# johannesulf/TabCorr

Hardware: AMD Instinct MI355X
Metric: predict_calls_per_sec (higher is better)
Workload: dtype f64; 1 GPU; BASELINE configs[1]: Zheng07 predict(), synthetic auto table 50 mass bins x {cen,sat} (G=100, P=5050), 19 rp bins, n_gauss_prim=10, batch of 10000 draws per GPU per step, draws and results resident in HBM; n_tables=1, gather=none, gather_payload=ngal + xi (160 B per draw), gather_every_steps=32, lanes=4, rccl_ranks=0

## Files before the change

tabcorr_amd/csrc/hostmath.cpp:

```cpp
#include "hostmath.h"
#include "fastmath.h"
#include "series.h"

#include <algorithm>
#include <atomic>
#include <cmath>
#include <cstring>
#include <map>
#include <numeric>
#include <tuple>
#include <thread>

namespace tc {

void gauss_legendre(int n, std::vector<double>& x, std::vector<double>& w) {
  x.assign(n, 0.0);
  w.assign(n, 0.0);
  const long double pi = 3.141592653589793238462643383279502884L;
  for (int i = 0; i < (n + 1) / 2; ++i) {
    long double z = cosl(pi * (i + 0.75L) / (n + 0.5L));
    long double dp = 1.0L;
    for (int iter = 0; iter < 100; ++iter) {
      long double p0 = 1.0L, p1 = z;
      for (int k = 2; k <= n; ++k) {
// ... 704 lines not shown
}

void triangle_parts(int n_rb, int n_parts, int32_t* rb0, int32_t* cb0, int32_t* count) {
  const int64_t n_units = (int64_t)n_rb * (n_rb + 1) / 2;
  for (int part = 0; part < n_parts; ++part) {
    const int64_t begin = n_units * part / n_parts, end = n_units * (part + 1) / n_parts;
    int64_t rb = (int64_t)((std::sqrt(8.0 * (double)begin + 1.0) - 1.0) / 2.0);
    while ((rb + 1) * (rb + 2) / 2 <= begin) ++rb;
    while (rb * (rb + 1) / 2 > begin) --rb;
    rb0[part] = (int32_t)rb;
    cb0[part] = (int32_t)(begin - rb * (rb + 1) / 2);
    count[part] = (int32_t)(end - begin);
  }
}

QuadTiling quad_tiling(int n_r) {
  QuadTiling tiling;
  tiling.n_rtiles = (n_r + 19) / 20;
  tiling.r_per_tile = (n_r + tiling.n_rtiles - 1) / tiling.n_rtiles;
  tiling.n_u = (tiling.r_per_tile + 3) / 4;
  return tiling;
}

void fill_quad_table(const QuadLayout& layout, const std::vector<int32_t>& perm, int n_r,
                     int64_t n_pairs, const void* matrix, bool matrix_is_f32,
                     const QuadTiling& tiling, std::vector<double>& out) {
  const int up = (tiling.n_u + 1) / 2;
  const size_t per_unit = (size_t)up * 128;
  out.assign((size_t)tiling.n_rtiles * layout.n_units * per_unit, 0.0);
  auto source = [&](int r, int64_t column) {
// ... 478 lines not shown
```

tabcorr_amd/csrc/hostmath.h:

```cpp
#pragma once

#include <cstdint>
#include <string>
#include <vector>

namespace tc {

void gauss_legendre(int n, std::vector<double>& x, std::vector<double>& w);

inline int64_t packed_index(int64_t i, int64_t j) {
  return i >= j ? i * (i + 1) / 2 + j : j * (j + 1) / 2 + i;
}

bool spline_interpolation_matrix(int n, const double* xp, std::vector<double>& a);

struct Segment {
  int32_t component;
  int32_t rectangular;
  int32_t i_lo, i_hi;
  int32_t j_lo, j_hi;
  int64_t q_begin;
  int64_t n_real;
};

// ... 114 lines not shown
  int32_t pad;
};
struct QuadMergePlan {
  int waves_per_block = 0;
  int n_blocks = 0;
  int lds_slots = 0;
  std::vector<int32_t> block_begin;
  std::vector<QuadMerge> merges;
};
void merge_quad_schedule(const QuadLayout& layout, int n_rtiles, bool separate,
                         int waves_per_block, int max_slots, QuadSchedule& schedule,
                         QuadMergePlan& plan);

void triangle_parts(int n_rb, int n_parts, int32_t* rb0, int32_t* cb0, int32_t* count);

struct QuadTiling {
  int n_rtiles = 1;
  int r_per_tile = 0;
  int n_u = 0;
};
QuadTiling quad_tiling(int n_r);

void fill_quad_table(const QuadLayout& layout, const std::vector<int32_t>& perm, int n_r,
                     int64_t n_pairs, const void* matrix, bool matrix_is_f32,
                     const QuadTiling& tiling, std::vector<double>& out);

QuadTiling quad_tiling_f32(int n_r);
void fill_quad_table_f32(const QuadLayout& layout, const std::vector<int32_t>& perm, int n_r,
                         int64_t n_pairs, const void* matrix, bool matrix_is_f32,
                         const QuadTiling& tiling, std::vector<float>& out);
// ... 47 lines not shown
```

tabcorr_amd/csrc/inst_fused.hip:

```cpp
#include "inst_fused.h"

namespace tc {
namespace host {

int launch_fused_instance(const FusedInstance& in, int device, int n_u, dim3 grid, dim3 block,
                       int lds, hipStream_t stream, hipEvent_t k0, hipEvent_t k1,
                       const tc::FusedArgs& fa) {
  const bool assembias = in.assembias, modulate = in.modulate;
  if (in.draws == 40) return launch_fused_instance_40(in, TC_FUSED_ARGS);
  if (in.draws == 32) return launch_fused_instance_32(in, TC_FUSED_ARGS);
  if (in.waves == 16) return launch_fused_instance_16(in, TC_FUSED_ARGS);
#define TC_FUSED(NG, AB, MO, LE) launch_fused<NG, AB, MO, LE, 8>(TC_FUSED_ARGS)
#define TC_FUSED_GROUPED(AB, MO) launch_fused<10, AB, MO, false, 8, 64, true>(TC_FUSED_ARGS)
  if (in.grouped)
    return assembias ? (modulate ? TC_FUSED_GROUPED(true, true) : TC_FUSED_GROUPED(true, false))
                     : (modulate ? TC_FUSED_GROUPED(false, true) : TC_FUSED_GROUPED(false, false));
  if (in.leauthaud) return modulate ? TC_FUSED(0, false, true, true) : TC_FUSED(0, false, false, true);
  if (in.n_gauss != 10) return TC_FUSED(0, false, false, false);
  if (!assembias && !modulate && in.defer == 2)
    return launch_fused<10, false, false, false, 8, 64, false, 2>(TC_FUSED_ARGS);
  if (!assembias && !modulate && in.defer == 1)
    return launch_fused<10, false, false, false, 8, 64, false, 1>(TC_FUSED_ARGS);
  if (!assembias && !modulate) return TC_FUSED(10, false, false, false);
  if (!assembias) return TC_FUSED(10, false, true, false);
  if (!modulate) return TC_FUSED(10, true, false, false);
  return TC_FUSED(10, true, true, false);
#undef TC_FUSED
#undef TC_FUSED_GROUPED
}

}
}
```

tabcorr_amd/csrc/internal.h:

```cpp
#pragma once

#include <hip/hip_runtime.h>
#include <hip/hip_ext.h>

#include <algorithm>
#include <chrono>
#include <cmath>
#include <cstdarg>
#include <cstdio>
#include <cstdlib>
#include <cstring>
#include <map>
#include <memory>
#include <string>
#include <utility>
#include <vector>

#include "../../include/tabcorr_amd.h"
#include "../../include/tabcorr_amd_testing.h"
#include "fastmath.h"
#include "hostmath.h"
#include "kernel_args.h"

namespace tc {
// ... 217 lines not shown
  int occ_splits = 0;
  int occ_per_cu = 4;
  int n_groups = 0, n_waves = 0, lds_min = 0, min_chunk_entries = 32;
  int k_splits = 0;
  int trace = 0;
  int autotune_after = 0;
  int sync_chunks = 0;
  int sync_form = 32;
  int sync_stagger = 10;
  int sync_direct_out = 2;
  int async_direct_in = 1;
  int async_direct_out = 2;
  int series = -1;
  int cross_defer = 1;
  int fused_defer = 2;
  int fused_sat_cap = 6;
  int cross_wide_min_draws = 4096;
  int cross_target = 160;
  int resident_aperture = 1;
  int cross_min_draws = 192;
  int fused = 1;
  int fused_min_draws = 0;
  int fused_max_draws = 30720;
  int fused_waves = 0;
  int fused_draws = 0;
  int fused_spread = 1, fused_spread_min = 8192, fused_spread_rounds = 1;
  int prio_fused = 1, prio_fused_occ = 2, prio_fused_out = 3;
  int deterministic = 0;
  int skip_occ = 0, skip_finalize = 0;
  void load() {
// ... 65 lines not shown
  int compute_dtype = TC_DTYPE_F64;
  bool legacy = false;
  tc::Plan plan;
  int rt = 0;
  int n_rtiles = 0;
  hipStream_t stream = nullptr;
  hipEvent_t ev_begin = nullptr, ev_end = nullptr;

  std::vector<double> n_h, log_min, log_max, percentile, dist_index;

  void* d_table = nullptr;
  size_t table_bytes = 0;
  void* d_n_h = nullptr;
  void* d_percentile = nullptr;
  void* d_perm = nullptr;
  tc::NodeGroups node_groups;
  void* d_group_begin = nullptr;
  void* d_group_member = nullptr;
  void* d_group_n_h = nullptr;
  void* d_group_percentile = nullptr;
  bool grouped = false;
  void* d_math_table = nullptr;
  void* d_pos_ij = nullptr;
  void* d_pos_off = nullptr;
  std::vector<double> cross_host;
  tc::host::CrossFused cross_fused, cross_fused_wide;
  int sync_cross_target = 0;
  std::vector<hipEvent_t> chunk_events;
  bool sync_spread = false;
  bool quad = false;
// ... 5 lines not shown
  std::map<unsigned, AutoChoice> autotuned;
  std::map<unsigned, int> pipelined_calls;
  bool autotuning = false;
  std::map<int, tc::host::Quadrature> quadrature;
  std::map<std::pair<int, int>, std::unique_ptr<tc::host::DeviceChunking>> chunkings;
  std::map<int64_t, tc::host::DeviceChunking*> choices;

  struct Lane {
    hipStream_t stream = nullptr;
    hipEvent_t finished = nullptr;
    tc::host::DeviceBuffer nbuf, ngal2, partial;
    tc::host::DeviceBuffer nbuf32;
    tc::host::DeviceBuffer xi;
    tc::host::DeviceBuffer in_theta, out;
    tc::host::DeviceBuffer cross_counters;
    int ngal_parts = 1;
  };
  static constexpr int kMaxLanes = 8;
  Lane lanes[kMaxLanes];
  int n_lanes = 2;
  int prev = -1;
  int cur = 0;
  int force_lane = -1;
  int async_lane = -1;
  bool chain = false;
  struct Ticket {
    hipEvent_t done = nullptr;
    int64_t id = -1;
  };
  static constexpr int kMaxTickets = 64;
// ... 161 lines not shown
int launch_occupation(const tc::OccArgs& oa, unsigned flags, int n_gauss, bool grouped,
                      int64_t grid_blocks, hipStream_t stream);
int launch_occ_from_array_kernel(const double* occupation_device, int64_t n_draws, int64_t ldb,
                                 int n_bins, int n_central, const double* n_h,
                                 const int32_t* perm, double* nbuf, double* ngal2, float* nbuf32,
                                 hipStream_t stream);
struct FusedInstance {
  int n_gauss = 10;
  bool assembias = false, modulate = false, leauthaud = false, grouped = false;
  int waves = 8, draws = 64;
  int defer = 0;
};
int launch_fused_instance(const FusedInstance& instance, int device, int n_u, dim3 grid,
                          dim3 block, int lds, hipStream_t stream, hipEvent_t k0, hipEvent_t k1,
                          const tc::FusedArgs& fa);
int launch_cross_instance(bool assembias, bool modulate, bool defer, int device, int rows,
                          dim3 grid, dim3 block, int lds, hipStream_t stream, hipEvent_t k0,
                          hipEvent_t k1, const tc::CrossFusedArgs& ca);
int launch_single_kernel(int blocks, hipStream_t stream, const tc::SingleArgs& sa);
int launch_resident_kernel(int blocks, hipStream_t stream, const tc::SingleArgs& sa);
int launch_ensemble_kernel(int device, int grid, int lds_bytes, hipStream_t stream,
                           const tc::EnsembleArgs& ea);

int copy_in(PinnedBuffer* stage, void* device, const void* host, size_t bytes,
            hipStream_t stream);
int copy_out(PinnedBuffer* stage, double* ngal, size_t ngal_count, const void* d_ngal,
             double* xi, size_t xi_count, const void* d_xi, hipStream_t stream);

}
}
// ... 1 lines not shown
```

tabcorr_amd/csrc/kernel_args.h:

```cpp
#pragma once

#include <cstdint>

#include "hostmath.h"

namespace tc {

constexpr int kLanes = 64;
constexpr unsigned kFlagSeparate = 1u;
constexpr unsigned kFlagModulate = 2u;
constexpr unsigned kFlagAssembias = 4u;
constexpr int kOccWaves = 4;
constexpr int kF32Block = 8;
constexpr int kF64Block = 8;
constexpr int kF32Tile = 32;
constexpr int kFinalizeRows = 32;
constexpr int kMaxInterpDim = 8;
constexpr int kMaxInterpAxis = 32;

struct GroupArgs {
  const int32_t* begin;
  const int32_t* member;
  const double* log_m;
  const double* m;
// ... 245 lines not shown
  uint32_t table_bytes;
  double* ngal;
  double* xi;
  const double* chi2_data;
  double* chi2;
  int n_groups;
  int n_central_groups;
  GroupArgs group;
  const double* series;
  const int32_t* series_thr;
  const double* sat_series;
  const int32_t* sat_series_thr;
  int sat_cap;
  const double* sat_records;
  const double* cen_records;
};

constexpr int kCrossWaves = 8;
constexpr int kCrossChunkBins = 48;
constexpr int kCrossMaxRows = 128;
constexpr int kCrossTableDoubles = 2306;
constexpr int kCrossSmallRows = 16, kCrossSmallChunk = 8;
constexpr int kCrossMaxSplits = 8;
constexpr int cross_small_lds_doubles(int n_comp) {
  return kCrossTableDoubles + kCrossWaves * kCrossSmallChunk * kLanes +
         n_comp * kCrossSmallRows * kLanes;
}
constexpr int cross_buffer_doubles(int rows) {
  return 2 * kCrossChunkBins * kLanes > rows * kLanes ? 2 * kCrossChunkBins * kLanes
                                                      : rows * kLanes;
// ... 87 lines not shown
```

tabcorr_amd/csrc/kernels.hip.h:

```cpp
#pragma once

#include <hip/hip_runtime.h>

#include <cstdint>
#include <utility>

#include "fastmath.h"
#include "hostmath.h"
#include "kernel_args.h"
#include "series.h"

#ifdef TC_DEVELOPER_KNOBS
#define TC_TRACE(pointer) ((pointer) != nullptr)
#else
#define TC_TRACE(pointer) false
#endif

namespace tc {

static_assert(sizeof(QuadRun) == 32 && sizeof(QuadCompArgs) == 32, "read as 8 x int32");

typedef const __attribute__((address_space(4))) double* sc_f64;
typedef const __attribute__((address_space(4))) float* sc_f32;
typedef const __attribute__((address_space(4))) int32_t* sc_i32;
// ... 1807 lines not shown
    }
    for (int idx = threadIdx.x; idx < rows * kLanes; idx += blockDim.x) {
      const int d = idx / rows, rr = idx % rows;
      if (d < n_valid) a.xi[(col + d) * (int64_t)n_rows + row0 + rr] = tile[rr][d];
    }
    __syncthreads();
  }
}

constexpr int fused_slot_doubles(int waves, int draws = 64) {
  return waves * 4 * kQuadMaxU * (draws == 40 ? 40 : kQuadTile);
}
__device__ __forceinline__ constexpr int dens40(int row, int draw) {
  return row * 40 + (draw & 3) * 10 + (draw >> 2);
}
constexpr int fused_scratch_doubles(int waves) { return fm::kTableDoubles + 2 * waves * kLanes; }
static_assert(kFusedWaves == 8 && kFusedMaxParts == 8, "8 or 16 waves: 4 or 8 parts per tile");
static_assert(20 * (kLanes + 1) + 20 * 21 <= fm::kTableDoubles,
              "results tile + likelihood data in the place of the math table");

template <int UU, int DL>
__device__ __forceinline__ void fused_quad_pass(__amdgpu_buffer_rsrc_t rs_t, unsigned off_a,
                                                unsigned unit_bytes, const double* dens_b,
                                                const double* dens_e, int rb, int cb, int left,
                                                bool triangular, int n_cb, unsigned unit_base,
                                                double (&F)[2][2]) {
  unsigned ua = (unit_base + (unsigned)(triangular ? rb * (rb + 1) / 2 + cb : rb * n_cb + cb)) *
                unit_bytes;
  f64x2 t0, t1, b0, b1;
  f64x4 D[UU][2];
  auto fetch = [&](f64x2& t, f64x2& b, int column) {
// ... 66 lines not shown
__device__ __forceinline__ int wave_prefix_sum(int value) {
  auto shifted = [](int x, auto control, auto rows) {
    return __builtin_amdgcn_update_dpp(0, x, decltype(control)::value, decltype(rows)::value, 0xf,
                                       false);
  };
  typedef std::integral_constant<int, 0xf> all_rows;
  value += shifted(value, std::integral_constant<int, 0x111>(), all_rows());
  value += shifted(value, std::integral_constant<int, 0x112>(), all_rows());
  value += shifted(value, std::integral_constant<int, 0x114>(), all_rows());
  value += shifted(value, std::integral_constant<int, 0x118>(), all_rows());
  value += shifted(value, std::integral_constant<int, 0x142>(), std::integral_constant<int, 0xa>());
  value += shifted(value, std::integral_constant<int, 0x143>(), std::integral_constant<int, 0xc>());
  return value;
}

__device__ __forceinline__ double fused_quad_rows40(double select, double value, double sums) {
  return __builtin_amdgcn_mfma_f64_4x4x4f64(select, value, sums, 0, 0, 0);
}

template <int S0, int NS>
__device__ __forceinline__ void fused_quad_pass40(__amdgpu_buffer_rsrc_t rs_t, unsigned off_a,
                                                  unsigned unit_bytes, const double* dens_b,
                                                  const double* dens_e, int rb, int cb, int left,
                                                  bool triangular, int n_cb, unsigned unit_base,
                                                  double (&F)[NS][10]) {
  unsigned ua = (unit_base + (unsigned)(triangular ? rb * (rb + 1) / 2 + cb : rb * n_cb + cb)) *
                unit_bytes;
  double ta[2][NS];
  f64x2 tb[2][5];
  double D[NS][10];
// ... 86 lines not shown

template <int NGAUSS, int U, bool ASSEMBIAS, bool MODULATE, bool LEAUTHAUD = false,
          int W = kFusedWaves, int DL = 64, bool GROUPED = false, int SATDEFER = 0>
__global__ __launch_bounds__(64 * W, DL == 40 ? 2 : W == 8 ? (SATDEFER == 2 ? 4 : 2) : 1) void predict_fused_kernel(
    FusedArgs a) {
  static_assert(!SATDEFER || (NGAUSS == 10 && !ASSEMBIAS && !MODULATE && !LEAUTHAUD && DL != 32 &&
                              !GROUPED), "deferred pairs");
  static_assert(!GROUPED || (NGAUSS == 10 && !LEAUTHAUD), "groups of bins: Zheng07, ten nodes");
  static_assert((DL == 64 && (W == 8 || W == 16)) || ((DL == 32 || DL == 40) && W == 8),
                "workgroup shape");
  static_assert(DL == 64 || NGAUSS == 10 || LEAUTHAUD, "32 / 40 draws: ten nodes per bin");
  static_assert(DL != 40 || (!ASSEMBIAS && !MODULATE && !LEAUTHAUD && !GROUPED), "latency form");
  constexpr int PARTS = DL == 40 ? W : W * 32 / DL;
  static_assert(!LEAUTHAUD || (NGAUSS == 0 && !ASSEMBIAS), "Leauthaud11: any n_gauss, undecorated");
  constexpr int UP = (U + 1) / 2;
  extern __shared__ __attribute__((aligned(16))) double fused_lds[];
  constexpr int kSlotDoubles = fused_slot_doubles(W, DL);
  const int region_b = a.dens_rows * DL > kSlotDoubles ? a.dens_rows * DL : kSlotDoubles;
  double* dens = fused_lds;
  double* table = fused_lds + region_b;
  double(*red)[W][kLanes] = (double(*)[W][kLanes])(table + fm::kTableDoubles);
  const fm::Consts kc = fm::make_consts();
#ifdef TC_DEVELOPER_KNOBS
  const int skip = (a.priority >> 8) & 3;
  const int n_bins_occ = (skip & 1) ? 0 : a.n_bins;
  unsigned long long* const stamps =
      ((a.priority >> 10) & 1) && a.chi2 == nullptr ? (unsigned long long*)a.chi2_data : nullptr;
  auto wave_stamp = [&](int which) {
    if (stamps != nullptr && (threadIdx.x & 63) == 0 && W == 8 && ((threadIdx.x >> 6) & 3) == 0)
      stamps[blockIdx.x * 32 + 16 + 8 * (threadIdx.x >> 8) + which] =
          __builtin_amdgcn_s_memrealtime();
  };
  auto stamp = [&](int which) {
    if (stamps != nullptr && threadIdx.x == 0)
      stamps[blockIdx.x * 32 + which] = __builtin_amdgcn_s_memrealtime();
  };
// ... 7 lines not shown
#endif
  stamp(0);
  set_priority((a.priority >> 2) & 3);
  const int lane = threadIdx.x & 63;
  const int wave = __builtin_amdgcn_readfirstlane(threadIdx.x >> 6);
  const int n_gauss = NGAUSS > 0 ? NGAUSS : a.n_gauss;
  {
    typedef double __attribute__((ext_vector_type(2))) double2v;
    const int hi = fm::kTableDoubles / 2;
    const double2v* src = (const double2v*)a.math_table;
    double2v* dst = (double2v*)table;
    for (int i = threadIdx.x; i < hi; i += blockDim.x) dst[i] = src[i];
  }
  for (int idx = a.n_bins * DL + threadIdx.x; idx < a.dens_rows * DL; idx += blockDim.x)
    dens[idx] = 0.0;
  __syncthreads();
  stamp(1);

  const int draw = DL != 32 ? lane : (lane & 31);
  const int half = DL != 32 ? 0 : (lane >> 5);
  const bool live = DL != 40 || lane < 40;
  auto dens_at = [&](int row, int d) -> double& {
    return dens[DL == 40 ? dens40(row, d) : row * DL + d];
  };
  const int64_t col = (int64_t)blockIdx.x * DL;
  const int64_t b0 = col + draw;
  const int64_t b = b0 < a.n_draws ? b0 : a.n_draws - 1;
  double norm;
  {
    const double* th = a.theta + b * a.n_theta;
    LeauthaudDraw ld;
    if (LEAUTHAUD) ld = prepare_leauthaud(table, kc, th);
    const DrawSetup d =
        LEAUTHAUD ? prepare_draw(table, kc, 12.0, 1.0, 12.0, 13.0, 1.0, 0.0, 0.0)
                  : prepare_draw(table, kc, th[0], th[1], th[2], th[3], th[4],
                                 ASSEMBIAS ? th[5] : 0.0, ASSEMBIAS ? th[6] : 0.0);
    DrawParams dp;
    dp.log_m_min = d.log_m_min;
    dp.inv_sigma = d.inv_sigma;
    dp.m0 = d.m0;
    dp.log2_m1 = d.log2_m1;
    dp.sat_scale = d.sat_scale;
// ... 27 lines not shown
          const double value = acc * n_h_m[mi];
          if (half == 0) dens[g * DL + draw] = value;
          if (central) sum_cen += value; else sum_sat += value;
        };
        if (DL == 32)
          occ_group_zheng07_halves<ASSEMBIAS, MODULATE>(
              table, kc, gr, group_begin[gr], group_begin[gr + 1], central, half, a.group.log_m,
              a.group.m, a.group.weight, gq, a.split, dp, emit);
        else
          occ_group_zheng07<ASSEMBIAS, MODULATE>(table, kc, gr, group_begin[gr],
                                                 group_begin[gr + 1], central, gq, a.split, dp,
                                                 emit);
      }
    }
    unsigned mine = 0;
    for (int g = wave; g < (GROUPED ? 0 : n_bins_occ); g += W) {
      const bool central = g < a.n_central;
      const bool above = ASSEMBIAS ? percentile[g] > a.split : false;
      bool deferred = false;
      const double acc =
          SATDEFER == 2 && central
              ? occ_cen_record(table, kc,
                               (sc_f64)a.cen_records + g * series::cen_record::kStride, dp,
                               &deferred) :
          SATDEFER && !central && (SATDEFER == 2 || a.sat_cap == series::sat::kShortest)
              ? occ_sat_record(table, kc,
                               (sc_f64)a.sat_records + g * series::sat_record::kStride, dp,
                               &deferred) :
          DL == 32 && LEAUTHAUD
              ? occ_bin_leauthaud11_halves<MODULATE>(table, kc, g, central, half, a.log_m, a.m,
// ... 2 lines not shown
                                                                    half, a.log_m, a.m, a.weight,
                                                                    log_m, weight_sum, dp)
          : LEAUTHAUD ? occ_bin_leauthaud11<MODULATE>(table, kc, g, n_gauss, central, log_m, mass,
                                                      weight, ld)
                      : occ_bin_zheng07<NGAUSS, ASSEMBIAS, MODULATE>(
                            table, kc, g, n_gauss, central, above, log_m, mass, weight,
                            weight_sum, dp, f1, f2,
                            SeriesConsts{(sc_f64)a.series, (sc_i32)a.series_thr, (sc_f64)a.sat_series,
                              (sc_i32)a.sat_series_thr,
                              SATDEFER ? a.sat_cap : series::sat::kSteps - 1},
                            SATDEFER ? &deferred : nullptr);
      if (SATDEFER && deferred && live) mine |= 1u << ((g - wave) / W);
      const double value = acc * n_h[g];
      if (half == 0 && live) dens_at(g, draw) = value;
      if (central) sum_cen += value; else sum_sat += value;
    }
    wave_stamp(0);
    if (SATDEFER) {
      unsigned* list = (unsigned*)&red[1][wave][0];
      const int count = __builtin_popcount(mine);
      const int inclusive = wave_prefix_sum(count);
      const int total = __builtin_amdgcn_readlane(inclusive, 63);
      wave_stamp(2);
      for (int base = 0; base < total; base += 64) {
        {
          unsigned left = mine;
          int position = inclusive - count - base;
          while (__builtin_amdgcn_ballot_w64(left != 0) != 0) {
            if (left != 0) {
              const int j = __builtin_ctz(left);
// ... 55 lines not shown
                      fm::exp2_fast(table, kc,
                                    alpha * fm::log2_fast_offset(
                                                table, kc, x > 1e-300 ? x : 1e-300, log2_m1),
                                    x > 0.0),
                      sat);
          }
        }
        sat *= sat_scale;
        if (bad != 0) {
          if ((bad & kInfSat) && sat != 0.0) sat = __builtin_huge_val();
          if ((bad & kBadSat) && sat != 0.0) sat = __builtin_nan("");
        }
        if (!cen_pair) acc = sat;
        }
        if (active) dens_at(g, from) = acc * a.n_h[g];
        wave_stamp(4);
      }
      for (unsigned left = mine; __builtin_amdgcn_ballot_w64(left != 0) != 0;) {
        if (left != 0) {
          const int j = __builtin_ctz(left);
          left &= left - 1;
          const double value = dens_at(wave + W * j, draw);
          if (SATDEFER == 2 && wave + W * j < a.n_central) sum_cen += value;
          else sum_sat += value;
        }
      }
    }
    wave_stamp(1);
    stamp(3);
    red[0][wave][lane] = sum_cen;
    red[1][wave][lane] = sum_sat;
    __syncthreads();
    stamp(4);
    double n_cen = 0.0, n_sat = 0.0;
#pragma unroll
    for (int w = 0; w < W; ++w) {
      n_cen += red[0][w][lane];
      n_sat += red[1][w][lane];
    }
    const double total = (skip & 1) ? 1.0 : n_cen + n_sat;
    norm = total * total;
    if (wave == 0 && half == 0 && live && b0 < a.n_draws) {
      if (a.separate) {
        a.ngal[2 * b0] = n_cen;
        a.ngal[2 * b0 + 1] = n_sat;
      } else {
// ... 39 lines not shown
    if (U > 3 && !(skip & 2))
      fused_quad_pass40<(U > 3 ? 3 : 0), UB>(rs_t, off_a, unit_bytes, dens_b, dens_e, rb, cb,
                                             count, triangular, n_cb, first_unit, F40b);
  } else {
    const int sub = wave / PARTS, part = wave % PARTS;
    const unsigned off_a = lane * 16;
    const double* dens_b =
        dens + (a.part_j_row0[part] + kq) * DL + sub * kQuadTile + 2 * c;
    const double* dens_e = dens + a.part_i_row0[part] * DL + sub * kQuadTile + 2 * c;
    const __amdgpu_buffer_rsrc_t rs_t =
        __builtin_amdgcn_make_buffer_rsrc((void*)a.table, 0, a.table_bytes, kBufferFlags);
    const int rb = a.part_rb0[part], cb = a.part_cb0[part], count = a.part_count[part];
    const bool triangular = a.part_triangular[part] != 0;
    const int n_cb = a.part_n_cb[part];
    const unsigned unit_base = (unsigned)a.part_unit_base[part];
#pragma unroll
    for (int p = 0; p < UP; ++p) {
      F[p][0][0] = F[p][0][1] = F[p][1][0] = F[p][1][1] = 0.0;
      if (skip & 2) continue;
      if (2 * p + 1 < U)
        fused_quad_pass<2, DL>(rs_t, off_a + p * 1024, UP * 1024, dens_b, dens_e, rb, cb, count,
                               triangular, n_cb, unit_base, F[p]);
      else
        fused_quad_pass<1, DL>(rs_t, off_a + p * 1024, UP * 1024, dens_b, dens_e, rb, cb, count,
                               triangular, n_cb, unit_base, F[p]);
    }
  }
  stamp(5);
  __syncthreads();
  stamp(8);
  if (DL == 40) {
    const int q = lane >> 4;
    auto share = [&](int sub, int g) {
      return sub < UA ? F40a[sub < UA ? sub : 0][g] : F40b[sub >= UA ? sub - UA : 0][g];
// ... 69 lines not shown
      double sum = first[0];
#pragma unroll
      for (int part = 1; part < W; ++part) sum += first[part * (4 * U) * 40];
      tile[rr][lane] = sum / norm;
    }
  } else {
    const int sub = lane >> 5, d = lane & 31;
    for (int rr = wave; rr < a.n_r && lane < DL; rr += W) {
      const double* first = dens + ((PARTS * sub) * (4 * U) + rr) * kQuadTile + d;
      double sum = first[0];
#pragma unroll
      for (int part = 1; part < PARTS; ++part) sum += first[part * (4 * U) * kQuadTile];
      tile[rr][lane] = sum / norm;
    }
  }
  __syncthreads();
  stamp(6);
  const int64_t n_valid = a.n_draws - col < DL ? a.n_draws - col : DL;
  if (a.chi2 != nullptr) {
    const int rows = a.n_r;
    const double* data = chi2_lds;
    const double* matrix = chi2_lds + rows;
    double part = 0.0;
    for (int i = wave; i < rows; i += W) {
      double inner = 0.0;
      for (int j = 0; j < rows; ++j)
        inner = fma(matrix[i * rows + j], tile[j][lane] - data[j], inner);
      part = fma(tile[i][lane] - data[i], inner, part);
    }
    red[0][wave][lane] = part;
    __syncthreads();
    if (wave == 0 && lane < n_valid) {
      double total = 0.0;
      for (int w = 0; w < W; ++w) total += red[0][w][lane];
      a.chi2[col + lane] = total;
    }
    return;
  }
  for (int idx = threadIdx.x; idx < a.n_r * DL; idx += blockDim.x) {
    const int d = idx / a.n_r, rr = idx % a.n_r;
    if (d < n_valid) a.xi[(col + d) * (int64_t)a.n_r + rr] = tile[rr][d];
  }
  stamp(7);
}

template <int ROW_LANES, typename Coefficient>
__device__ __forceinline__ void cross_deferred_pairs(
    const CrossFusedArgs& a, const double* table, const fm::Consts& kc, const DrawParams& dp,
    const unsigned long long* bitmap, unsigned* list, int wave, int lane, int g_first, int g_last,
    int type, Coefficient&& coefficient, double* res) {
  constexpr int SHARES = 64 / ROW_LANES;
  constexpr int SLOTS = 8 / SHARES;
  const int row = lane % ROW_LANES, share = lane / ROW_LANES;
  const unsigned long long owner = 0x0101010101010101ull << wave;
  double extra[SLOTS];
#pragma unroll
// ... 1817 lines not shown
```

tabcorr_amd/csrc/launch.hip:

```cpp
#include <immintrin.h>

#include <atomic>
#include <mutex>

#include "internal.h"
#include "kernels.hip.h"
#include "series.h"

namespace tc {
namespace host {

int get_quadrature(tc_table* t, int n_gauss, Quadrature** out) {
  auto it = t->quadrature.find(n_gauss);
  if (it != t->quadrature.end()) {
    *out = &it->second;
    return TC_OK;
  }
  std::vector<double> x, w;
  tc::gauss_legendre(n_gauss, x, w);
  const int g = t->n_bins;
  std::vector<double> log_m((size_t)g * n_gauss), m((size_t)g * n_gauss),
      weight((size_t)g * n_gauss + g);
  for (int i = 0; i < g; ++i) {
    const double d_log = t->log_max[i] - t->log_min[i];
// ... 1023 lines not shown
  if (sat_defer) fa.sat_series = (const double*)q->sat_series;
  fa.sat_records = (const double*)q->sat_records;
  fa.cen_records = (const double*)q->cen_records;
  const bool cen_defer = sat_defer && t->tuning.fused_defer >= 2 && (series_mask(t) & 1) != 0 &&
                         q->cen_records != nullptr;
  fa.sat_cap = t->tuning.fused_sat_cap;
  tc::host::FusedInstance instance{};
  instance.n_gauss = n_gauss == 10 ? 10 : 0;
  instance.assembias = assembias;
  instance.modulate = modulate;
  instance.leauthaud = (flags & TC_FLAG_LEAUTHAUD11) != 0;
  instance.waves = waves;
  instance.draws = draws;
  instance.grouped = t->grouped && n_gauss == 10 && !(flags & TC_FLAG_LEAUTHAUD11);
  instance.defer = cen_defer ? 2 : sat_defer ? 1 : 0;
  status = launch_fused_instance(instance, t->device, t->quad_tiling.n_u, grid, block, lds, stream,
                                 k0, k1, fa);
  if (status != TC_OK) return status;
  t->last_workgroups = (int)grid.x;
  t->last_waves = waves;
  t->last_splits = 0;
  t->last_lds = lds;
  t->prev = t->force_lane >= 0 ? -1 : t->cur;
  return TC_OK;
}


CrossFused* choose_cross_fused(tc_table* const* tables, int n_tables, CrossFused* narrow,
                               CrossFused* wide, int64_t n_draws, unsigned flags, int* status) {
  const tc_table* t0 = tables[0];
// ... 930 lines not shown
```

tabcorr_amd/csrc/table.cpp:

```cpp
#include <cmath>

#include "internal.h"

using namespace tc::host;

extern "C" {

int tc_table_create(int mode, int n_bins, int n_r, int64_t n_pairs,
                    const void* tpcf_matrix, int matrix_dtype, const double* n_h,
                    const double* log_min, const double* log_max,
                    const double* percentile, const double* dist_index,
                    const uint8_t* is_central, int compute_dtype, tc_table** out) {
  TC_CHECK(out != nullptr, "table output pointer is NULL");
  *out = nullptr;
  TC_CHECK(mode == TC_MODE_AUTO || mode == TC_MODE_CROSS, "invalid mode %d", mode);
  TC_CHECK(n_bins >= 1 && n_bins < (1 << 20), "invalid number of bins %d", n_bins);
  TC_CHECK(n_r >= 1, "invalid number of correlation function bins %d", n_r);
  const int64_t expect =
      mode == TC_MODE_AUTO ? (int64_t)n_bins * (n_bins + 1) / 2 : n_bins;
  TC_CHECK(n_pairs == expect,
           "tpcf_matrix has %lld columns but %d bins in mode '%s' need %lld",
           (long long)n_pairs, n_bins, mode == TC_MODE_AUTO ? "auto" : "cross",
           (long long)expect);
  TC_CHECK(n_pairs < (1LL << 31), "too many pair columns");
// ... 169 lines not shown

int tc_table_destroy(tc_table* t) {
  if (t == nullptr) return TC_OK;
  (void)hipSetDevice(t->device);
  (void)resident_stop(t);
  if (t->resident.stream) (void)hipStreamDestroy(t->resident.stream);
  t->resident.mailbox.release();
  t->resident.ens_mailbox.release();
  t->resident.ens_out.release();
  t->resident.ens_device.release();
  t->resident.ens_aperture.release();
  t->resident.single_aperture.release();
  t->resident.ws.buffer.release();
  for (tc_table::Lane& lane : t->lanes)
    if (lane.stream) (void)hipStreamSynchronize(lane.stream);
  for (void* p : {t->d_table, t->d_n_h, t->d_percentile, t->d_perm, t->d_math_table,
                  t->d_pos_ij, t->d_pos_off, t->d_group_begin, t->d_group_member,
                  t->d_group_n_h, t->d_group_percentile})
    if (p) (void)hipFree(p);
  for (auto& kv : t->quadrature)
    for (void* p : {kv.second.log_m, kv.second.m, kv.second.weight, kv.second.group_log_m,
                    kv.second.group_m, kv.second.group_weight, kv.second.series,
                    kv.second.series_thr, kv.second.group_series, kv.second.group_series_thr,
                    kv.second.sat_series, kv.second.sat_series_thr, kv.second.group_sat_series,
                    kv.second.group_sat_series_thr, kv.second.group_records, kv.second.sat_records, kv.second.cen_records})
      if (p) (void)hipFree(p);
  for (auto& kv : t->chunkings)
    for (void* p : {kv.second->chunks, kv.second->groups})
      if (p) (void)hipFree(p);
  t->quad_by_type.release();
  t->quad_total.release();
  t->cross_fused.release();
  t->cross_fused_wide.release();
  for (DeviceBuffer* b : {&t->theta, &t->out_ngal, &t->out_xi, &t->occupation,
                          &t->trace, &t->wave_trace, &t->chi2_data})
    b->release();
  for (tc_table::Lane& lane : t->lanes) {
    lane.nbuf.release();
    lane.ngal2.release();
    lane.partial.release();
    lane.xi.release();
    lane.nbuf32.release();
    lane.in_theta.release();
    lane.out.release();
    lane.cross_counters.release();
    if (lane.finished) (void)hipEventDestroy(lane.finished);
  }
  for (tc_table::Ticket& ticket : t->tickets)
    if (ticket.done) (void)hipEventDestroy(ticket.done);
  t->h_in.release();
  t->h_out.release();
  t->single_ws.buffer.release();
  for (auto& ev : t->kernel_events) {
    (void)hipEventDestroy(ev.first);
    (void)hipEventDestroy(ev.second);
  }
  for (hipEvent_t event : t->chunk_events) (void)hipEventDestroy(event);
  if (t->ev_begin) (void)hipEventDestroy(t->ev_begin);
  if (t->ev_end) (void)hipEventDestroy(t->ev_end);
  for (tc_table::Lane& lane : t->lanes)
// ... 1044 lines not shown
  } else if (key == "resident_aperture") {
    TC_CHECK(value == 0 || value == 1, "resident_aperture must be 0 or 1");
    const int status = resident_stop(t);
    if (status != TC_OK) return status;
    t->tuning.resident_aperture = value;
    t->resident.ens_grid = 0;
    t->resident.single_aperture_decided = false;
  } else if (key == "cross_min_draws") {
    TC_CHECK(value >= 1, "cross_min_draws must be positive");
    t->tuning.cross_min_draws = value;
  } else if (key == "cross_defer") {
    t->tuning.cross_defer = value != 0;
  } else if (key == "fused_defer") {
    TC_CHECK(value >= 0 && value <= 2, "fused_defer must be 0, 1 or 2");
    t->tuning.fused_defer = value;
  } else if (key == "fused_sat_cap") {
    TC_CHECK(value >= 0 && value <= 6, "fused_sat_cap must be in [0, 6]");
    t->tuning.fused_sat_cap = value;
  } else if (key == "cross_wide_min_draws") {
    TC_CHECK(value >= 0, "cross_wide_min_draws must not be negative");
    t->tuning.cross_wide_min_draws = value;
  } else if (key == "cross_target") {
    TC_CHECK(value >= 1 && value <= 4096, "cross_target must be in [1, 4096]");
    t->tuning.cross_target = value;
  } else if (key == "series") {
    TC_CHECK(value >= -1 && value <= 3, "series must be -1 .. 3");
    t->tuning.series = value;
  } else if (key == "grouped") {
    t->grouped = value != 0 && t->node_groups.largest > 1;
  } else if (key == "lanes") {
// ... 215 lines not shown
```

Measured before the change: 272.5 million calls/s.

## Sort draws by satellite mass key and skip empty quadratic-form rows

Adds a pre-pass kernel that buckets draws by which satellite mass block their log M0 falls in, so each 64-draw tile holds draws with similar nonzero occupation rows. The fused kernel then records which density row blocks are nonzero per tile and walks only those rows and columns of the triangular quadratic form, with a precomputed load-balanced row split across four parts. Outputs are scattered back through the permutation. This adds an extra launch, an indirect gather of theta and a scattered write of results. The skip is disabled when values are too large, but it still relies on exact zeros in the densities.

```diff
diff --git a/tabcorr_amd/csrc/hostmath.cpp b/tabcorr_amd/csrc/hostmath.cpp
--- a/tabcorr_amd/csrc/hostmath.cpp
+++ b/tabcorr_amd/csrc/hostmath.cpp
@@ -742,6 +742,24 @@
   }
 }
 
+void fused_row_parts(int n_rb, int first_sat_row, uint64_t* rows) {
+  int64_t load[4] = {0, 0, 0, 0};
+  for (int part = 0; part < 4; ++part) rows[part] = 0;
+  first_sat_row = std::max(0, std::min(first_sat_row, n_rb));
+  for (int rb = first_sat_row; rb < n_rb; ++rb) {
+    const int part = (rb - first_sat_row) % 4;
+    rows[part] |= (uint64_t)1 << rb;
+    load[part] += rb + 1;
+  }
+  for (int rb = first_sat_row - 1; rb >= 0; --rb) {
+    int part = 0;
+    for (int other = 1; other < 4; ++other)
+      if (load[other] < load[part]) part = other;
+    rows[part] |= (uint64_t)1 << rb;
+    load[part] += rb + 1;
+  }
+}
+
 QuadTiling quad_tiling(int n_r) {
   QuadTiling tiling;
   tiling.n_rtiles = (n_r + 19) / 20;
diff --git a/tabcorr_amd/csrc/hostmath.h b/tabcorr_amd/csrc/hostmath.h
--- a/tabcorr_amd/csrc/hostmath.h
+++ b/tabcorr_amd/csrc/hostmath.h
@@ -152,6 +152,8 @@
 
 void triangle_parts(int n_rb, int n_parts, int32_t* rb0, int32_t* cb0, int32_t* count);
 
+void fused_row_parts(int n_rb, int first_sat_row, uint64_t* rows);
+
 struct QuadTiling {
   int n_rtiles = 1;
   int r_per_tile = 0;
diff --git a/tabcorr_amd/csrc/inst_fused.hip b/tabcorr_amd/csrc/inst_fused.hip
--- a/tabcorr_amd/csrc/inst_fused.hip
+++ b/tabcorr_amd/csrc/inst_fused.hip
@@ -29,5 +29,13 @@
 #undef TC_FUSED_GROUPED
 }
 
+int launch_fused_group(hipStream_t stream, const tc::GroupDrawsArgs& ga) {
+  hipLaunchKernelGGL(tc::fused_group_kernel<tc::kGroupWaves>, dim3(tc::kGroupBlocks),
+                     dim3(64 * tc::kGroupWaves),
+                     0, stream, ga);
+  TC_HIP(hipGetLastError());
+  return TC_OK;
+}
+
 }
 }
diff --git a/tabcorr_amd/csrc/internal.h b/tabcorr_amd/csrc/internal.h
--- a/tabcorr_amd/csrc/internal.h
+++ b/tabcorr_amd/csrc/internal.h
@@ -255,6 +255,7 @@
   int series = -1;
   int cross_defer = 1;
   int fused_defer = 2;
+  int fused_skip = 1;
   int fused_sat_cap = 6;
   int cross_wide_min_draws = 4096;
   int cross_target = 160;
@@ -350,6 +351,8 @@
   void* d_n_h = nullptr;
   void* d_percentile = nullptr;
   void* d_perm = nullptr;
+  void* d_sat_edges = nullptr;
+  int n_sat_edges = -1;
   tc::NodeGroups node_groups;
   void* d_group_begin = nullptr;
   void* d_group_member = nullptr;
@@ -385,6 +388,7 @@
     tc::host::DeviceBuffer xi;
     tc::host::DeviceBuffer in_theta, out;
     tc::host::DeviceBuffer cross_counters;
+    tc::host::DeviceBuffer draw_order;
     int ngal_parts = 1;
   };
   static constexpr int kMaxLanes = 8;
@@ -576,6 +580,7 @@
 int launch_fused_instance(const FusedInstance& instance, int device, int n_u, dim3 grid,
                           dim3 block, int lds, hipStream_t stream, hipEvent_t k0, hipEvent_t k1,
                           const tc::FusedArgs& fa);
+int launch_fused_group(hipStream_t stream, const tc::GroupDrawsArgs& ga);
 int launch_cross_instance(bool assembias, bool modulate, bool defer, int device, int rows,
                           dim3 grid, dim3 block, int lds, hipStream_t stream, hipEvent_t k0,
                           hipEvent_t k1, const tc::CrossFusedArgs& ca);
diff --git a/tabcorr_amd/csrc/kernel_args.h b/tabcorr_amd/csrc/kernel_args.h
--- a/tabcorr_amd/csrc/kernel_args.h
+++ b/tabcorr_amd/csrc/kernel_args.h
@@ -283,6 +283,22 @@
   int sat_cap;
   const double* sat_records;
   const double* cen_records;
+  unsigned long long part_rows[4];
+  int skip;
+  const int32_t* perm;
+};
+
+constexpr int kGroupWaves = 16;
+constexpr int kGroupBlocks = 8;
+constexpr int kGroupMaxKeys = 64;
+constexpr int kGroupMaxDraws = 32768;
+struct GroupDrawsArgs {
+  const double* theta;
+  int n_theta;
+  int n_edges;
+  int64_t n_draws;
+  const double* edges;
+  int32_t* perm;
 };
 
 constexpr int kCrossWaves = 8;
diff --git a/tabcorr_amd/csrc/kernels.hip.h b/tabcorr_amd/csrc/kernels.hip.h
--- a/tabcorr_amd/csrc/kernels.hip.h
+++ b/tabcorr_amd/csrc/kernels.hip.h
@@ -1845,7 +1845,9 @@
 __device__ __forceinline__ constexpr int dens40(int row, int draw) {
   return row * 40 + (draw & 3) * 10 + (draw >> 2);
 }
-constexpr int fused_scratch_doubles(int waves) { return fm::kTableDoubles + 2 * waves * kLanes; }
+constexpr int fused_scratch_doubles(int waves) {
+  return fm::kTableDoubles + 2 * waves * kLanes + 4;
+}
 static_assert(kFusedWaves == 8 && kFusedMaxParts == 8, "8 or 16 waves: 4 or 8 parts per tile");
 static_assert(20 * (kLanes + 1) + 20 * 21 <= fm::kTableDoubles,
               "results tile + likelihood data in the place of the math table");
@@ -1942,6 +1944,169 @@
   return value;
 }
 
+template <int UU, int DL>
+__device__ __forceinline__ void fused_quad_rows(__amdgpu_buffer_rsrc_t rs_t, unsigned off_a,
+                                                unsigned unit_bytes, const double* dens_b,
+                                                const double* dens_e, unsigned long long rows,
+                                                unsigned long long live, unsigned unit_base,
+                                                double (&F)[2][2]) {
+  rows &= live;
+  if (rows == 0) return;
+  f64x2 t0, t1, b0, b1;
+  f64x4 D[UU][2];
+  auto fetch = [&](f64x2& t, f64x2& b, int row, int column) {
+    t = buffer_load16<0>(rs_t, off_a, (unit_base + (unsigned)(row * (row + 1) / 2 + column)) * unit_bytes);
+    b = *(const f64x2*)(dens_b + 4 * column * DL);
+  };
+  auto mma = [&](const f64x2& t, const f64x2& b, bool first) {
+    if (first) {
+      const f64x4 zero = {0.0, 0.0, 0.0, 0.0};
+#pragma unroll
+      for (int u = 0; u < UU; ++u) {
+        const double av = u ? t.y : t.x;
+        D[u][0] = __builtin_amdgcn_mfma_f64_16x16x4f64(av, b.x, zero, 0, 0, 0);
+        D[u][1] = __builtin_amdgcn_mfma_f64_16x16x4f64(av, b.y, zero, 0, 0, 0);
+      }
+    } else {
+#pragma unroll
+      for (int u = 0; u < UU; ++u) {
+        const double av = u ? t.y : t.x;
+        D[u][0] = __builtin_amdgcn_mfma_f64_16x16x4f64(av, b.x, D[u][0], 0, 0, 0);
+        D[u][1] = __builtin_amdgcn_mfma_f64_16x16x4f64(av, b.y, D[u][1], 0, 0, 0);
+      }
+    }
+  };
+  const int c0 = __builtin_ctzll(live);
+  int rb = __builtin_ctzll(rows);
+  fetch(t0, b0, rb, c0);
+  while (true) {
+    rows &= rows - 1;
+    const int rb_next = rows != 0 ? __builtin_ctzll(rows) : rb;
+    unsigned long long cols = live & (~0ull >> (63 - rb));
+    const int n = __builtin_popcountll(cols);
+    cols &= cols - 1;
+    auto next_column = [&]() {
+      const int column = __builtin_ctzll(cols);
+      cols &= cols - 1;
+      return column;
+    };
+    f64x2 e[4];
+#pragma unroll
+    for (int v = 0; v < 4; ++v) e[v] = *(const f64x2*)(dens_e + (4 * rb + v) * DL);
+    if (n > 1) fetch(t1, b1, rb, next_column()); else fetch(t1, b1, rb_next, c0);
+    __builtin_amdgcn_sched_barrier(0);
+    mma(t0, b0, true);
+    __builtin_amdgcn_sched_barrier(0);
+    int t = 1;
+    for (; t + 1 < n; t += 2) {
+      fetch(t0, b0, rb, next_column());
+      __builtin_amdgcn_sched_barrier(0);
+      mma(t1, b1, false);
+      __builtin_amdgcn_sched_barrier(0);
+      if (t + 2 < n) fetch(t1, b1, rb, next_column()); else fetch(t1, b1, rb_next, c0);
+      __builtin_amdgcn_sched_barrier(0);
+      mma(t0, b0, false);
+      __builtin_amdgcn_sched_barrier(0);
+    }
+    if (t < n) {
+      fetch(t0, b0, rb_next, c0);
+      __builtin_amdgcn_sched_barrier(0);
+      mma(t1, b1, false);
+      __builtin_amdgcn_sched_barrier(0);
+    } else {
+      t0 = t1;
+      b0 = b1;
+    }
+#pragma unroll
+    for (int u = 0; u < UU; ++u)
+#pragma unroll
+      for (int v = 0; v < 4; ++v) {
+        F[u][0] = fma(D[u][0][v], e[v].x, F[u][0]);
+        F[u][1] = fma(D[u][1][v], e[v].y, F[u][1]);
+      }
+    if (rows == 0) break;
+    rb = rb_next;
+  }
+}
+
+template <int WAVES>
+__global__ __launch_bounds__(64 * WAVES) void fused_group_kernel(GroupDrawsArgs a) {
+  static_assert(WAVES == kGroupWaves, "kernel_args.h");
+  constexpr int SHARES = kGroupWaves * kGroupBlocks;
+  __shared__ int start[SHARES][kGroupMaxKeys];
+  __shared__ int total[kGroupMaxKeys];
+  __shared__ double edges[kGroupMaxKeys];
+  __shared__ unsigned char keys[kGroupMaxDraws];
+  const int lane = threadIdx.x & 63;
+  const int wave = __builtin_amdgcn_readfirstlane(threadIdx.x >> 6);
+  const int n_keys = a.n_edges + 1;
+  set_priority(3);
+  for (int i = threadIdx.x; i < SHARES * kGroupMaxKeys; i += blockDim.x) (&start[0][0])[i] = 0;
+  for (int i = threadIdx.x; i < a.n_edges; i += blockDim.x) edges[i] = a.edges[i];
+  __syncthreads();
+#pragma unroll 4
+  for (int draw = threadIdx.x; draw < (int)a.n_draws; draw += blockDim.x) {
+    const double* th = a.theta + (int64_t)draw * a.n_theta;
+    bool finite = true;
+    for (int i = 0; i < a.n_theta; ++i) finite = finite && fabs(th[i]) <= 1.79769313486231570815e308;
+    const double log_m0 = th[2];
+    int lo = 0, hi = a.n_edges;
+    while (lo < hi) {
+      const int mid = (lo + hi) >> 1;
+      if (edges[mid] <= log_m0) lo = mid + 1; else hi = mid;
+    }
+    keys[draw] = (unsigned char)(finite ? lo : 0);
+  }
+  __syncthreads();
+  const int share = (int)(((a.n_draws + SHARES - 1) / SHARES + 63) / 64 * 64);
+  for (int s = wave; s < SHARES; s += kGroupWaves) {
+    const int begin = share * s;
+    const int end = begin + share < (int)a.n_draws ? begin + share : (int)a.n_draws;
+    for (int base = begin; base < end; base += 64)
+      if (base + lane < end) atomicAdd(&start[s][keys[base + lane]], 1);
+  }
+  __syncthreads();
+  for (int k = threadIdx.x; k < n_keys; k += blockDim.x) {
+    int sum = 0;
+    for (int s = 0; s < SHARES; ++s) sum += start[s][k];
+    total[k] = sum;
+  }
+  __syncthreads();
+  if (wave == 0) {
+    const int count = lane < n_keys ? total[lane] : 0;
+    const int inclusive = wave_prefix_sum(count);
+    if (lane < n_keys) total[lane] = inclusive - count;
+  }
+  __syncthreads();
+  for (int k = threadIdx.x; k < n_keys; k += blockDim.x) {
+    int at = total[k];
+    for (int s = 0; s < SHARES; ++s) {
+      const int count = start[s][k];
+      start[s][k] = at;
+      at += count;
+    }
+  }
+  __syncthreads();
+  const int mine = (int)blockIdx.x * kGroupWaves + wave;
+  int next = lane < n_keys ? start[mine][lane] : 0;
+  const int begin = share * mine;
+  const int end = begin + share < (int)a.n_draws ? begin + share : (int)a.n_draws;
+  for (int base = begin; base < end; base += 64) {
+    const bool valid = base + lane < end;
+    const int key = valid ? (int)keys[base + lane] : -1;
+    unsigned long long todo = __builtin_amdgcn_ballot_w64(valid);
+    while (todo != 0) {
+      const int k = __builtin_amdgcn_readlane(key, __builtin_ctzll(todo));
+      const unsigned long long same = __builtin_amdgcn_ballot_w64(key == k);
+      const int at = __builtin_amdgcn_readlane(next, k);
+      if (key == k)
+        a.perm[at + __builtin_popcountll(same & ((1ull << lane) - 1))] = (int32_t)(base + lane);
+      if (lane == k) next += __builtin_popcountll(same);
+      todo &= ~same;
+    }
+  }
+}
+
 __device__ __forceinline__ double fused_quad_rows40(double select, double value, double sums) {
   return __builtin_amdgcn_mfma_f64_4x4x4f64(select, value, sums, 0, 0, 0);
 }
@@ -2058,12 +2223,14 @@
   constexpr int PARTS = DL == 40 ? W : W * 32 / DL;
   static_assert(!LEAUTHAUD || (NGAUSS == 0 && !ASSEMBIAS), "Leauthaud11: any n_gauss, undecorated");
   constexpr int UP = (U + 1) / 2;
+  constexpr bool ROWS = SATDEFER != 0 && DL == 64 && W == 8;
   extern __shared__ __attribute__((aligned(16))) double fused_lds[];
   constexpr int kSlotDoubles = fused_slot_doubles(W, DL);
   const int region_b = a.dens_rows * DL > kSlotDoubles ? a.dens_rows * DL : kSlotDoubles;
   double* dens = fused_lds;
   double* table = fused_lds + region_b;
   double(*red)[W][kLanes] = (double(*)[W][kLanes])(table + fm::kTableDoubles);
+  unsigned long long* const live_lds = (unsigned long long*)(table + fm::kTableDoubles + 2 * W * kLanes);
   const fm::Consts kc = fm::make_consts();
 #ifdef TC_DEVELOPER_KNOBS
   const int skip = (a.priority >> 8) & 3;
@@ -2101,6 +2268,7 @@
   }
   for (int idx = a.n_bins * DL + threadIdx.x; idx < a.dens_rows * DL; idx += blockDim.x)
     dens[idx] = 0.0;
+  if (ROWS && threadIdx.x < 3) live_lds[threadIdx.x] = 0;
   __syncthreads();
   stamp(1);
 
@@ -2111,8 +2279,11 @@
     return dens[DL == 40 ? dens40(row, d) : row * DL + d];
   };
   const int64_t col = (int64_t)blockIdx.x * DL;
-  const int64_t b0 = col + draw;
-  const int64_t b = b0 < a.n_draws ? b0 : a.n_draws - 1;
+  const int64_t place = col + draw;
+  const bool grouped_draws = ROWS && a.perm != nullptr && !a.separate;
+  const int64_t last = place < a.n_draws ? place : a.n_draws - 1;
+  const int64_t b = grouped_draws ? (int64_t)a.perm[last] : last;
+  const int64_t b0 = place < a.n_draws ? b : a.n_draws;
   double norm;
   {
     const double* th = a.theta + b * a.n_theta;
@@ -2170,6 +2341,8 @@
       }
     }
     unsigned mine = 0;
+    unsigned long long live0 = 0, live1 = 0;
+    unsigned full = 0;
     for (int g = wave; g < (GROUPED ? 0 : n_bins_occ); g += W) {
       const bool central = g < a.n_central;
       const bool above = ASSEMBIAS ? percentile[g] > a.split : false;
@@ -2202,6 +2375,13 @@
       const double value = acc * n_h[g];
       if (half == 0 && live) dens_at(g, draw) = value;
       if (central) sum_cen += value; else sum_sat += value;
+      if (ROWS) {
+        const unsigned long long nonzero = __builtin_amdgcn_ballot_w64(value != 0.0 || deferred);
+        const unsigned long long wild = __builtin_amdgcn_ballot_w64(!(fabs(value) <= 1e140));
+        if ((unsigned)nonzero != 0) live0 |= 1ull << (g >> 2);
+        if ((nonzero >> 32) != 0) live1 |= 1ull << (g >> 2);
+        full |= ((unsigned)wild != 0 ? 1u : 0u) | ((wild >> 32) != 0 ? 2u : 0u);
+      }
     }
     wave_stamp(0);
     if (SATDEFER) {
@@ -2287,6 +2467,12 @@
         if (!cen_pair) acc = sat;
         }
         if (active) dens_at(g, from) = acc * a.n_h[g];
+        if (ROWS) {
+          const unsigned long long wild =
+              __builtin_amdgcn_ballot_w64(active && !(fabs(acc * a.n_h[g]) <= 1e140));
+          const unsigned long long second = __builtin_amdgcn_ballot_w64(from >= 32);
+          full |= ((wild & ~second) != 0 ? 1u : 0u) | ((wild & second) != 0 ? 2u : 0u);
+        }
         wave_stamp(4);
       }
       for (unsigned left = mine; __builtin_amdgcn_ballot_w64(left != 0) != 0;) {
@@ -2303,6 +2489,11 @@
     stamp(3);
     red[0][wave][lane] = sum_cen;
     red[1][wave][lane] = sum_sat;
+    if (ROWS && lane == 0) {
+      atomicOr(&live_lds[0], live0);
+      atomicOr(&live_lds[1], live1);
+      atomicOr(&live_lds[2], (unsigned long long)full);
+    }
     __syncthreads();
     stamp(4);
     double n_cen = 0.0, n_sat = 0.0;
@@ -2372,10 +2563,32 @@
     const bool triangular = a.part_triangular[part] != 0;
     const int n_cb = a.part_n_cb[part];
     const unsigned unit_base = (unsigned)a.part_unit_base[part];
+    const bool by_rows = ROWS && !a.separate;
+    unsigned long long part_rows = 0, live_blocks = 0;
+    if (by_rows) {
+      const unsigned long long every = ~0ull >> (64 - n_cb);
+      const unsigned long long seen =
+          __builtin_amdgcn_readfirstlane((unsigned)live_lds[sub]) |
+          ((unsigned long long)__builtin_amdgcn_readfirstlane((unsigned)(live_lds[sub] >> 32)) << 32);
+      const unsigned wild = __builtin_amdgcn_readfirstlane((unsigned)live_lds[2]);
+      const bool may_skip =
+          a.skip != 0 && !(skip & 1) && ((a.priority >> 11) & 1) && !((wild >> sub) & 1);
+      live_blocks = may_skip ? (seen & every) : every;
+      part_rows = a.part_rows[part & 3];
+    }
 #pragma unroll
     for (int p = 0; p < UP; ++p) {
       F[p][0][0] = F[p][0][1] = F[p][1][0] = F[p][1][1] = 0.0;
       if (skip & 2) continue;
+      if (by_rows) {
+        if (2 * p + 1 < U)
+          fused_quad_rows<2, DL>(rs_t, off_a + p * 1024, UP * 1024, dens_b, dens_e, part_rows,
+                                 live_blocks, unit_base, F[p]);
+        else
+          fused_quad_rows<1, DL>(rs_t, off_a + p * 1024, UP * 1024, dens_b, dens_e, part_rows,
+                                 live_blocks, unit_base, F[p]);
+        continue;
+      }
       if (2 * p + 1 < U)
         fused_quad_pass<2, DL>(rs_t, off_a + p * 1024, UP * 1024, dens_b, dens_e, rb, cb, count,
                                triangular, n_cb, unit_base, F[p]);
@@ -2475,6 +2688,8 @@
       tile[rr][lane] = sum / norm;
     }
   }
+  int* const places = (int*)&red[1][0][0];
+  if (grouped_draws && wave == 0) places[lane] = (int)b;
   __syncthreads();
   stamp(6);
   const int64_t n_valid = a.n_draws - col < DL ? a.n_draws - col : DL;
@@ -2494,13 +2709,14 @@
     if (wave == 0 && lane < n_valid) {
       double total = 0.0;
       for (int w = 0; w < W; ++w) total += red[0][w][lane];
-      a.chi2[col + lane] = total;
+      a.chi2[b0] = total;
     }
     return;
   }
   for (int idx = threadIdx.x; idx < a.n_r * DL; idx += blockDim.x) {
     const int d = idx / a.n_r, rr = idx % a.n_r;
-    if (d < n_valid) a.xi[(col + d) * (int64_t)a.n_r + rr] = tile[rr][d];
+    const int64_t out = grouped_draws ? (int64_t)places[d < n_valid ? d : 0] : col + d;
+    if (d < n_valid) a.xi[out * (int64_t)a.n_r + rr] = tile[rr][d];
   }
   stamp(7);
 }
diff --git a/tabcorr_amd/csrc/launch.hip b/tabcorr_amd/csrc/launch.hip
--- a/tabcorr_amd/csrc/launch.hip
+++ b/tabcorr_amd/csrc/launch.hip
@@ -1061,6 +1061,47 @@
   instance.draws = draws;
   instance.grouped = t->grouped && n_gauss == 10 && !(flags & TC_FLAG_LEAUTHAUD11);
   instance.defer = cen_defer ? 2 : sat_defer ? 1 : 0;
+  if (instance.defer != 0 && !separate) {
+    const tc::QuadComp& comp = q_table.layout.comps[0];
+    TC_CHECK(comp.n_rb <= 64, "the one-launch form's row split holds 64 block rows");
+    uint64_t rows[4];
+    tc::fused_row_parts(comp.n_rb, (t->plan.n_central + 3) / 4, rows);
+    for (int part = 0; part < 4; ++part) fa.part_rows[part] = rows[part];
+    fa.skip = t->tuning.fused_skip != 0 ? 1 : 0;
+    if (fa.skip && n_theta >= 3 && n_draws > 64 && n_draws <= tc::kGroupMaxDraws) {
+      if (t->n_sat_edges < 0) {
+        std::vector<double> edges;
+        for (int block = (t->plan.n_central + 3) / 4; 4 * block < t->n_bins; ++block) {
+          double top = t->log_max[4 * block];
+          for (int g = 4 * block; g < std::min(4 * block + 4, t->n_bins); ++g)
+            top = std::max(top, t->log_max[g]);
+          edges.push_back(top);
+        }
+        std::sort(edges.begin(), edges.end());
+        edges.erase(std::unique(edges.begin(), edges.end()), edges.end());
+        bool usable = (int)edges.size() < tc::kGroupMaxKeys;
+        for (const double edge : edges) usable = usable && std::isfinite(edge);
+        if (!usable) edges.clear();
+        status = upload(edges, &t->d_sat_edges);
+        if (status != TC_OK) return status;
+        t->n_sat_edges = (int)edges.size();
+      }
+      if (t->n_sat_edges > 0) {
+        status = lane.draw_order.reserve((size_t)n_draws * sizeof(int32_t), stream);
+        if (status != TC_OK) return status;
+        tc::GroupDrawsArgs ga{};
+        ga.theta = theta_device;
+        ga.n_theta = n_theta;
+        ga.n_edges = t->n_sat_edges;
+        ga.n_draws = n_draws;
+        ga.edges = (const double*)t->d_sat_edges;
+        ga.perm = (int32_t*)lane.draw_order.ptr;
+        status = launch_fused_group(stream, ga);
+        if (status != TC_OK) return status;
+        fa.perm = (const int32_t*)lane.draw_order.ptr;
+      }
+    }
+  }
   status = launch_fused_instance(instance, t->device, t->quad_tiling.n_u, grid, block, lds, stream,
                                  k0, k1, fa);
   if (status != TC_OK) return status;
diff --git a/tabcorr_amd/csrc/table.cpp b/tabcorr_amd/csrc/table.cpp
--- a/tabcorr_amd/csrc/table.cpp
+++ b/tabcorr_amd/csrc/table.cpp
@@ -207,7 +207,7 @@
   t->resident.ws.buffer.release();
   for (tc_table::Lane& lane : t->lanes)
     if (lane.stream) (void)hipStreamSynchronize(lane.stream);
-  for (void* p : {t->d_table, t->d_n_h, t->d_percentile, t->d_perm, t->d_math_table,
+  for (void* p : {t->d_table, t->d_n_h, t->d_percentile, t->d_perm, t->d_sat_edges, t->d_math_table,
                   t->d_pos_ij, t->d_pos_off, t->d_group_begin, t->d_group_member,
                   t->d_group_n_h, t->d_group_percentile})
     if (p) (void)hipFree(p);
@@ -237,6 +237,7 @@
     lane.in_theta.release();
     lane.out.release();
     lane.cross_counters.release();
+    lane.draw_order.release();
     if (lane.finished) (void)hipEventDestroy(lane.finished);
   }
   for (tc_table::Ticket& ticket : t->tickets)
@@ -1311,6 +1312,9 @@
   } else if (key == "fused_defer") {
     TC_CHECK(value >= 0 && value <= 2, "fused_defer must be 0, 1 or 2");
     t->tuning.fused_defer = value;
+  } else if (key == "fused_skip") {
+    TC_CHECK(value == 0 || value == 1, "fused_skip must be 0 or 1");
+    t->tuning.fused_skip = value;
   } else if (key == "fused_sat_cap") {
     TC_CHECK(value >= 0 && value <= 6, "fused_sat_cap must be in [0, 6]");
     t->tuning.fused_sat_cap = value;
```

After: 255.0 million calls/s. -6.4%, worse.
